# stsievert/pytorch-ps-mpi

Measured on AMD Instinct MI355X. Metric: samples/sec (node) ResNet-50 async PS at 1/2/4/8 MI355X; grad bytes/step, higher is better.
Workload: dtype bf16

## Files before the change

### hipps/csrc/bindings.cpp

```cpp
#include <torch/extension.h>
#include <vector>

namespace hipps {
void aggregate(const std::vector<at::Tensor>& slots, at::Tensor acc, double gscale, bool accumulate, bool acquire);
void copy_acquire(at::Tensor src, at::Tensor dst);
void convert(at::Tensor src, at::Tensor dst, double scale);
void gather_flat(const std::vector<at::Tensor>& srcs, at::Tensor table, at::Tensor dst, double scale);
void transpose_cast(at::Tensor src, at::Tensor dst, at::Tensor tiles);
void sgd_step(const std::vector<at::Tensor>& grads, double gscale, at::Tensor p, c10::optional<at::Tensor> buf,
              c10::optional<at::Tensor> pub, bool zero_src, double lr, double wd, double momentum, double dampening,
              bool nesterov, bool first, c10::optional<at::Tensor> mask, c10::optional<at::Tensor> csteps,
              double lookahead);
void adam_step(const std::vector<at::Tensor>& grads, double gscale, at::Tensor p, at::Tensor exp_avg,
               at::Tensor exp_avg_sq, c10::optional<at::Tensor> max_exp_avg_sq, c10::optional<at::Tensor> pub,
               bool zero_src, double lr, double beta1, double beta2, double eps, double wd, int64_t step,
               bool amsgrad, bool torch_mode, c10::optional<at::Tensor> mask, c10::optional<at::Tensor> csteps);
void q8_encode(at::Tensor x, c10::optional<at::Tensor> resid, at::Tensor q, at::Tensor scales, bool stochastic,
               int64_t seed);
void q8_aggregate(const std::vector<at::Tensor>& qs, const std::vector<at::Tensor>& ss, at::Tensor acc, double gscale,
                  bool accumulate, bool acquire);
void topk_encode(at::Tensor g, c10::optional<at::Tensor> resid, int64_t k, at::Tensor idx, at::Tensor val,
                 at::Tensor workspace);
int64_t topk_workspace_bytes(int64_t n, int64_t k);
void topk_accumulate(at::Tensor idx, at::Tensor val, at::Tensor acc, double gscale, bool acquire);
// ... 23 lines not shown
void bn_backward_partials(at::Tensor part, int64_t nrb, at::Tensor dy, at::Tensor x, int64_t mask_mode,
                          at::Tensor weight, at::Tensor mean, at::Tensor invstd, at::Tensor scale, at::Tensor shift,
                          at::Tensor dx, c10::optional<at::Tensor> dres, at::Tensor dweight, at::Tensor dbias, int64_t C,
                          c10::optional<at::Tensor> mask_in, int64_t unr);
int64_t conv1x1_mtiles(int64_t M);
void conv1x1_forward(at::Tensor x, at::Tensor w, at::Tensor y, c10::optional<at::Tensor> part, int64_t Hi,
                     int64_t Wi, int64_t stride, c10::optional<at::Tensor> add, c10::optional<at::Tensor> add_mask,
                     c10::optional<at::Tensor> bn_x, c10::optional<at::Tensor> bn_bits,
                     c10::optional<at::Tensor> bn_mean, c10::optional<at::Tensor> bn_invstd,
                     c10::optional<at::Tensor> bn_scale, c10::optional<at::Tensor> bn_shift,
                     c10::optional<at::Tensor> pro_scale, c10::optional<at::Tensor> pro_shift);
void bn_dual_forward(at::Tensor part3, int64_t nrb3, at::Tensor partd, int64_t nrbd, at::Tensor x3, at::Tensor xd,
                     at::Tensor z, at::Tensor mask, at::Tensor w3, at::Tensor b3, at::Tensor rm3, at::Tensor rv3,
                     at::Tensor mean3, at::Tensor invstd3, at::Tensor scale3, at::Tensor shift3, at::Tensor wd,
                     at::Tensor bd, at::Tensor rmd, at::Tensor rvd, at::Tensor meand, at::Tensor invstdd,
                     at::Tensor scaled, at::Tensor shiftd, int64_t C, double eps3, double mom3, double epsd,
                     double momd);
void bn_dual_backward(c10::optional<at::Tensor> part3, int64_t nrb3, at::Tensor dz, at::Tensor x3, at::Tensor xd,
                      at::Tensor mask, at::Tensor w3, at::Tensor mean3, at::Tensor invstd3, at::Tensor wd,
                      at::Tensor meand, at::Tensor invstdd, at::Tensor dx3, at::Tensor dxd, at::Tensor dw3,
                      at::Tensor db3, at::Tensor dwd, at::Tensor dbd, int64_t C, int64_t unr);
at::Tensor gemm2_dgrad_s2(at::Tensor dy, at::Tensor wf, at::Tensor dx, int64_t bm, int64_t bn,
                          c10::optional<at::Tensor> bn_x, c10::optional<at::Tensor> bn_bits,
                          c10::optional<at::Tensor> bn_mean, c10::optional<at::Tensor> bn_invstd,
                          c10::optional<at::Tensor> bn_scale, c10::optional<at::Tensor> bn_shift);
int64_t gemm2_mtiles(int64_t M, int64_t N, int64_t K, int64_t bm);
void gemm2_conv(at::Tensor x, at::Tensor w, at::Tensor y, c10::optional<at::Tensor> part,
                c10::optional<at::Tensor> add, c10::optional<at::Tensor> add_mask, int64_t Hi, int64_t Wi,
                int64_t stride, int64_t KH, int64_t KW, int64_t pad, int64_t bm, int64_t bn,
                c10::optional<at::Tensor> bn_x, c10::optional<at::Tensor> bn_bits, c10::optional<at::Tensor> bn_mean,
                c10::optional<at::Tensor> bn_invstd, c10::optional<at::Tensor> bn_scale,
                c10::optional<at::Tensor> bn_shift, int64_t stages, bool add_s2,
                c10::optional<at::Tensor> pro_scale, c10::optional<at::Tensor> pro_shift,
                c10::optional<at::Tensor> bias, c10::optional<at::Tensor> gelu_pre, int64_t gelu);
void gemm2_wgrad(at::Tensor dy, at::Tensor x, at::Tensor dw, int64_t KH, int64_t KW, int64_t stride, int64_t pad,
                 int64_t Hi, int64_t Wi, int64_t cfg, int64_t stages,
                 c10::optional<at::Tensor> pro_scale, c10::optional<at::Tensor> pro_shift, int64_t sdiv);
void maxpool3s2_forward(at::Tensor x, at::Tensor y, at::Tensor code, c10::optional<at::Tensor> scale,
                        c10::optional<at::Tensor> shift);
void bn_finalize_partials(at::Tensor part, int64_t nrb, int64_t M, at::Tensor weight, at::Tensor bias,
                          c10::optional<at::Tensor> running_mean, c10::optional<at::Tensor> running_var,
                          at::Tensor mean, at::Tensor invstd, at::Tensor scale, at::Tensor shift, int64_t C, double eps,
                          double momentum);
void maxpool3s2_backward(at::Tensor dy, at::Tensor code, at::Tensor dx);
std::vector<at::Tensor> xent_forward(at::Tensor logits, at::Tensor labels, int64_t ignore_index);
void colsum_fold(at::Tensor part, at::Tensor out);
void colsum_bf16(at::Tensor x, at::Tensor out);
std::vector<at::Tensor> attn_forward(at::Tensor q, at::Tensor k, at::Tensor v, bool causal, double scale,
                                     c10::optional<at::Tensor> kvlen);
std::vector<at::Tensor> attn_backward(at::Tensor dout, at::Tensor q, at::Tensor k, at::Tensor v, at::Tensor o,
                                      at::Tensor lse, bool causal, double scale, c10::optional<at::Tensor> kvlen,
                                      c10::optional<at::Tensor> dq_out, c10::optional<at::Tensor> dk_out,
                                      c10::optional<at::Tensor> dv_out);
void swiglu_forward(at::Tensor a, at::Tensor b, at::Tensor c);
void ln_forward(at::Tensor x, at::Tensor w, at::Tensor b, at::Tensor y, at::Tensor mean, at::Tensor rstd, double eps);
void ln_backward(at::Tensor dy, at::Tensor x, at::Tensor mean, at::Tensor rstd, at::Tensor w, at::Tensor dx,
                 at::Tensor dw, at::Tensor db, c10::optional<at::Tensor> dxsum);
void embed_forward(at::Tensor ids, c10::optional<at::Tensor> tt, at::Tensor word, at::Tensor pos, at::Tensor typ,
                   at::Tensor out);
void embed_pos_backward(at::Tensor dout, at::Tensor dpos, int64_t B, int64_t S);
void embed_seg_backward(at::Tensor dout, at::Tensor sid, at::Tensor perm, at::Tensor dtab);
void rms_forward(at::Tensor x, at::Tensor w, at::Tensor y, at::Tensor rstd, double eps, c10::optional<at::Tensor> add,
                 c10::optional<at::Tensor> xsum);
void rms_backward(at::Tensor dy, at::Tensor x, at::Tensor rstd, at::Tensor w, at::Tensor dx, at::Tensor dw,
                  c10::optional<at::Tensor> dres, c10::optional<at::Tensor> dx16);
void swiglu_backward(at::Tensor g, at::Tensor a, at::Tensor b, at::Tensor da, at::Tensor db);
void rope_apply(at::Tensor x, at::Tensor y, at::Tensor cs, at::Tensor sn, int64_t S, int64_t hd, double sign);
// ... 74 lines not shown
        py::arg("acc"), py::arg("gscale"), py::arg("acquire") = false);
  m.def("topk_q8_accumulate", &hipps::topk_q8_accumulate, "acc[idx] += gscale * deq(q)", py::arg("idx"), py::arg("q"),
        py::arg("scales"), py::arg("acc"), py::arg("gscale"), py::arg("acquire") = false);
  m.def("topk_q8_residual", &hipps::topk_q8_residual, "EF: r[idx] += v - deq(q)");
  m.def("thresh_encode", &hipps::thresh_encode, "variable-size |x|>tau sparsification, device count header");
  m.def("thresh_accumulate", &hipps::thresh_accumulate, "acc[idx[:count]] += gscale * val[:count]", py::arg("count"),
        py::arg("idx"), py::arg("val"), py::arg("acc"), py::arg("gscale"), py::arg("acquire") = false);
  m.def("copy_counted", &hipps::copy_counted, "copy a [count | idx | val] message moving only count entries");
  m.def("bn_forward_train", &hipps::bn_forward_train, "fused channels-last BN train fwd (+res) (+relu)");
  m.def("bn_apply", &hipps::bn_apply, "y = act(x*scale + shift (+res))");
  m.def("bn_backward", &hipps::bn_backward, "fused BN bwd with relu-mask recompute (+dres)");
  m.def("bn_forward_partials", &hipps::bn_forward_partials, "BN fwd finalize+apply from producer-reduced partials");
  m.def("bn_backward_partials", &hipps::bn_backward_partials, "BN bwd finalize+apply from consumer-reduced partials",
        py::arg("part"), py::arg("nrb"), py::arg("dy"), py::arg("x"), py::arg("mask_mode"), py::arg("weight"),
        py::arg("mean"), py::arg("invstd"), py::arg("scale"), py::arg("shift"), py::arg("dx"), py::arg("dres"),
        py::arg("dweight"), py::arg("dbias"), py::arg("C"), py::arg("mask_in"), py::arg("unr") = 0);
  m.def("conv1x1_mtiles", &hipps::conv1x1_mtiles);
  m.def("bn_dual_forward", &hipps::bn_dual_forward,
        "z = relu(bn3(x3) + bnd(xd)) from producer partials: two finalizes + one apply (downsample block)");
  m.def("bn_dual_backward", &hipps::bn_dual_backward,
        "backward of bn_dual_forward: dx3 + the downsample BN's reduction in one pass, then dxd",
        py::arg("part3"), py::arg("nrb3"), py::arg("dz"), py::arg("x3"), py::arg("xd"), py::arg("mask"), py::arg("w3"),
        py::arg("mean3"), py::arg("invstd3"), py::arg("wd"), py::arg("meand"), py::arg("invstdd"), py::arg("dx3"),
        py::arg("dxd"), py::arg("dw3"), py::arg("db3"), py::arg("dwd"), py::arg("dbd"), py::arg("C"),
        py::arg("unr") = 4);
  m.def("gemm2_mtiles", &hipps::gemm2_mtiles, py::arg("M"), py::arg("N"), py::arg("K"), py::arg("bm") = 0);
  m.def("gemm2_conv", &hipps::gemm2_conv, "second-generation MFMA conv GEMM (LDS-DMA staged, 256-row tiles)",
        py::arg("x"), py::arg("w"), py::arg("y"), py::arg("part") = py::none(), py::arg("add") = py::none(),
        py::arg("add_mask") = py::none(), py::arg("Hi"), py::arg("Wi"), py::arg("stride") = 1, py::arg("KH") = 1,
        py::arg("KW") = 1, py::arg("pad") = 0, py::arg("bm") = 0, py::arg("bn") = 0, py::arg("bn_x") = py::none(),
        py::arg("bn_bits") = py::none(), py::arg("bn_mean") = py::none(), py::arg("bn_invstd") = py::none(),
        py::arg("bn_scale") = py::none(), py::arg("bn_shift") = py::none(), py::arg("stages") = 2,
        py::arg("add_s2") = false, py::arg("pro_scale") = py::none(), py::arg("pro_shift") = py::none(),
        py::arg("bias") = py::none(), py::arg("gelu_pre") = py::none(), py::arg("gelu") = 0);
  m.def("gemm2_dgrad_s2", &hipps::gemm2_dgrad_s2,
        "stride-2 3x3 input gradient as four output-parity implicit GEMMs (+ BN-backward reduction)",
        py::arg("dy"), py::arg("wf"), py::arg("dx"), py::arg("bm") = 128, py::arg("bn") = 128,
        py::arg("bn_x") = py::none(), py::arg("bn_bits") = py::none(), py::arg("bn_mean") = py::none(),
        py::arg("bn_invstd") = py::none(), py::arg("bn_scale") = py::none(), py::arg("bn_shift") = py::none());
  m.def("gemm2_wgrad", &hipps::gemm2_wgrad, "conv weight gradient on the LDS-DMA MFMA core (split-M slabs)",
        py::arg("dy"), py::arg("x"), py::arg("dw"), py::arg("KH"), py::arg("KW"), py::arg("stride"), py::arg("pad"),
        py::arg("Hi"), py::arg("Wi"), py::arg("cfg") = 0, py::arg("stages") = 2, py::arg("pro_scale") = py::none(),
        py::arg("pro_shift") = py::none(), py::arg("sdiv") = 1);
  m.def("conv1x1_forward", &hipps::conv1x1_forward,
        "MFMA 1x1 conv (NHWC GEMM) with fused BN-stats epilogue and optional (+ add * mask) epilogue",
        pybind11::arg("x"), pybind11::arg("w"), pybind11::arg("y"), pybind11::arg("part"), pybind11::arg("Hi"),
        pybind11::arg("Wi"), pybind11::arg("stride"), pybind11::arg("add") = pybind11::none(),
        pybind11::arg("add_mask") = pybind11::none(), pybind11::arg("bn_x") = pybind11::none(),
        pybind11::arg("bn_bits") = pybind11::none(), pybind11::arg("bn_mean") = pybind11::none(),
        pybind11::arg("bn_invstd") = pybind11::none(), pybind11::arg("bn_scale") = pybind11::none(),
        pybind11::arg("bn_shift") = pybind11::none(), pybind11::arg("pro_scale") = pybind11::none(),
        pybind11::arg("pro_shift") = pybind11::none());
  m.def("convkxk_forward", &hipps::convkxk_forward,
        "MFMA KxK conv forward (implicit GEMM, channels-last bf16) with optional BN-statistics epilogue",
        pybind11::arg("x"), pybind11::arg("w"), pybind11::arg("y"), pybind11::arg("part") = pybind11::none(),
        pybind11::arg("stride") = 1, pybind11::arg("pad") = 1);
  m.def("stem_mtiles", &hipps::stem_mtiles, "number of BN partial-statistic columns of stem_forward");
  m.def("stem_forward", &hipps::stem_forward,
        "ResNet stem 7x7/s2/p3 3->64 conv forward on MFMA (channels-last bf16), optional BN-statistics epilogue",
        pybind11::arg("x"), pybind11::arg("w"), pybind11::arg("y"), pybind11::arg("part") = pybind11::none());
  m.def("stem_bnpool_backward", &hipps::stem_bnpool_backward,
        "backward of maxpool(relu(bn(stem(x)))): BN parameter grads + stem weight grad, no pool gradient "
        "materialised (the BN input gradient only with materialize_dy)",
        py::arg("dp"), py::arg("code"), py::arg("y"), py::arg("x"), py::arg("bn_weight"), py::arg("mean"),
        py::arg("invstd"), py::arg("scale"), py::arg("shift"), py::arg("dbn_w"), py::arg("dbn_b"), py::arg("dw"),
        py::arg("materialize_dy") = false, py::arg("quad") = true);
  m.def("stem_wgrad", &hipps::stem_wgrad, "ResNet stem 7x7/s2/p3 weight gradient on MFMA (fp32 dW, deterministic)");
// ... 82 lines not shown
```

### hipps/csrc/gemm2.hip

```cpp
#include "common.h"

#include <ATen/ATen.h>
#include <cstdlib>
#include <mutex>
#include <c10/hip/HIPStream.h>
#include <torch/extension.h>

namespace hipps {
namespace g2 {

typedef short bf16x8 __attribute__((ext_vector_type(8)));
typedef float f32x4 __attribute__((ext_vector_type(4)));
typedef float f32x16 __attribute__((ext_vector_type(16)));
typedef uint32_t u32x4 __attribute__((ext_vector_type(4)));
typedef __attribute__((address_space(3))) void lds_void;
typedef __attribute__((address_space(1))) void glb_void;

constexpr int BK = 64;

__device__ __attribute__((aligned(64))) const uint16_t kZero16[32] = {0};
__device__ __attribute__((aligned(64))) const uint8_t kOnes8[64] = {
    0xff, 0xff, 0xff, 0xff, 0xff, 0xff, 0xff, 0xff, 0xff, 0xff, 0xff, 0xff, 0xff, 0xff, 0xff, 0xff,
    0xff, 0xff, 0xff, 0xff, 0xff, 0xff, 0xff, 0xff, 0xff, 0xff, 0xff, 0xff, 0xff, 0xff, 0xff, 0xff,
    0xff, 0xff, 0xff, 0xff, 0xff, 0xff, 0xff, 0xff, 0xff, 0xff, 0xff, 0xff, 0xff, 0xff, 0xff, 0xff,
    0xff, 0xff, 0xff, 0xff, 0xff, 0xff, 0xff, 0xff, 0xff, 0xff, 0xff, 0xff, 0xff, 0xff, 0xff, 0xff};

enum Epi : int { kPlain = 0, kStats = 1, kAdd = 2, kBst = 4, kBstBits = 8, kAddS2 = 16, kPar = 32, kPro = 64,
                 kBias = 128, kGelu = 256, kGeluB = 512, kGeluBS = 1024 };

__device__ __forceinline__ float erf_fast(float z, float& ez2) {
  const float az = fabsf(z);
  const float t = __builtin_amdgcn_rcpf(fmaf(0.3275911f, az, 1.f));
  ez2 = __expf(-az * az);
  float p = fmaf(1.061405429f, t, -1.453152027f);
  p = fmaf(p, t, 1.421413741f);
  p = fmaf(p, t, -0.284496736f);
  p = fmaf(p, t, 0.254829592f);
  const float e = fmaf(-p * t, ez2, 1.f);
  return copysignf(e, z);
}
__device__ __forceinline__ float gelu_f(float x) {
  float ez2;
  return x * 0.5f * (1.f + erf_fast(x * 0.70710678118654752f, ez2));
}
__device__ __forceinline__ float gelu_bwd_f(float dy, float x) {
  float ez2;
  const float cdf = 0.5f * (1.f + erf_fast(x * 0.70710678118654752f, ez2));
  return dy * fmaf(x, 0.3989422804014327f * ez2, cdf);
}

template <int BM, int BN> struct Cfg;
template <> struct Cfg<256, 256> { static constexpr int TM = 128, TN = 64; };
template <> struct Cfg<256, 128> { static constexpr int TM = 64, TN = 64; };
template <> struct Cfg<128, 128> { static constexpr int TM = 64, TN = 64; };
template <> struct Cfg<256, 64> { static constexpr int TM = 64, TN = 64; };
template <> struct Cfg<128, 64> { static constexpr int TM = 64, TN = 32; };

template <int BM, int BN> constexpr int nthreads() { return 64 * (BM / Cfg<BM, BN>::TM) * (BN / Cfg<BM, BN>::TN); }

template <int BM, int BN, int NS = 2> constexpr int lds_bytes() {
  constexpr int stage = (NS >= 4 ? 2 : NS) * (BM + BN) * BK * 2;
  constexpr int epi = BM * (BN + 8) * 2;
  constexpr int wm = BM / Cfg<BM, BN>::TM;
  return (stage > epi ? stage : epi) + 2 * 2 * wm * BN * 4;
}

struct Args {
  const uint16_t* X;
  const uint16_t* W;
  uint16_t* Y;
  float* pa;
  float* pb;
  const uint16_t* R;
  const uint8_t* RM;
  const uint16_t* bx;
  const uint8_t* bbits;
  const float *bmean, *binvstd, *bscale, *bshift;
  int M, N, K, Ho, Wo, Hi, Wi, stride, mtiles, ntiles;
  int KW, pad, Cin;
  int ldb;
  int pstride, pcol0;
  int ph, pw, Hx, Wx;
  int tdr[4], tdc[4], tko[4];
  const float *psc, *psh;
  const float* bias;
  uint16_t* Y2;
  int epf;
};

__device__ __forceinline__ uint32_t add_bf16x2(uint32_t a, uint32_t b) {
  return pack_bf16x2(__uint_as_float(a << 16) + __uint_as_float(b << 16),
                     __uint_as_float(a & 0xffff0000u) + __uint_as_float(b & 0xffff0000u));
}

__device__ __forceinline__ void glds16(const void* src, void* dst) {
  __builtin_amdgcn_global_load_lds((glb_void*)src, (lds_void*)dst, 16, 0, 0);
}

constexpr int waitcnt_vm(int n) { return (n & 15) | ((n >> 4) << 14) | (7 << 4) | (15 << 8); }
constexpr int waitcnt_lgkm(int n) { return 15 | (3 << 14) | (7 << 4) | ((n & 15) << 8); }

__host__ __device__ constexpr int khalf_swz(int row) {
  return ((0x1320 >> (4 * ((row >> 2) & 3))) & 3);
}

template <int BM, int BN, int EPI, bool TAPS, int NS>
__global__ __launch_bounds__((nthreads<BM, BN>())) void k_gemm(Args g) {
  constexpr int TM = Cfg<BM, BN>::TM, TN = Cfg<BM, BN>::TN;
  constexpr int WM = BM / TM, WN = BN / TN, NW = WM * WN, NT = 64 * NW;
  constexpr int FM = TM / 16, FN = TN / 16;
  constexpr bool KH = NS == 4;
  constexpr bool PP = NS == 5;
  constexpr bool M32 = NS == 6;
  constexpr int NSX = M32 ? 2 : NS;
  constexpr bool PAR = (EPI & kPar) != 0;
  constexpr bool PRO = (EPI & kPro) != 0;
  static_assert(!PAR || TAPS, "kPar needs the implicit-GEMM loader");
  static_assert(!PRO || NS == 2, "kPro: 2 LDS stages");
  static_assert(!PP || (BM == 256 && BN == 256), "ping-pong: 256x256 on 8 waves");
  static_assert(!M32 || (BM == 256 && BN == 256 && !PRO), "32x32x16 MFMA: the 256x256 tile");
  auto orow = [&](int m) -> int64_t {
    if constexpr (PAR) {
      const int hw = g.Ho * g.Wo;
      const int img = m / hw, rem = m - img * hw;
      const int a = rem / g.Wo, b = rem - a * g.Wo;
      return ((int64_t)img * g.Hx + 2 * a + g.ph) * g.Wx + 2 * b + g.pw;
    } else {
      return m;
    }
  };
  constexpr int STAGE = (BM + BN) * BK;
  constexpr int UNIT = (BM + BN) * 32;
  constexpr int RPI = KH ? 16 : 8;
// ... 602 lines not shown
    float* red = reinterpret_cast<float*>(lds);
    __syncthreads();
#pragma unroll
    for (int j = 0; j < 8; ++j) {
      red[(t / RCH) * BN + cc + j] = bsa[j];
      red[RL * BN + (t / RCH) * BN + cc + j] = bsb[j];
    }
    __syncthreads();
    if (t < BN) {
      float sa = 0.f, sb = 0.f;
      for (int r = 0; r < RL; ++r) {
        sa += red[r * BN + t];
        sb += red[RL * BN + r * BN + t];
      }
      if constexpr (GBS) {
        g.pa[(int64_t)mt * g.N + n0 + t] = sa;
      } else {
        g.pa[(int64_t)(n0 + t) * g.pstride + g.pcol0 + mt] = sa;
        g.pb[(int64_t)(n0 + t) * g.pstride + g.pcol0 + mt] = sb;
      }
    }
  }
  if (STATS && t < BN) {
    float sa = 0.f, qa = 0.f;
#pragma unroll
    for (int i = 0; i < WM; ++i) {
      sa += st[(i * BN + t) * 2];
      qa += st[(i * BN + t) * 2 + 1];
    }
    g.pa[(int64_t)(n0 + t) * g.pstride + g.pcol0 + mt] = sa;
    g.pb[(int64_t)(n0 + t) * g.pstride + g.pcol0 + mt] = qa;
  }
}

struct FastDiv2 {
  uint32_t d, mul, shift;
};
inline FastDiv2 make_fastdiv2(uint32_t d) {
  uint32_t l = 0;
  while ((1ull << l) < d) ++l;
  const uint64_t mul = ((((1ull << l) - d) << 32) / d) + 1;
  return FastDiv2{d, (uint32_t)mul, l};
}
__device__ __forceinline__ uint32_t fdiv2(uint32_t n, const FastDiv2& f) { return (__umulhi(n, f.mul) + n) >> f.shift; }

struct WArgs {
  const uint16_t* dY;
  const uint16_t* X;
  float* part;
  int M, N, K, Cin, Ho, Wo, Hi, Wi, stride, KW, pad, chunk, tn, tk;
  FastDiv2 fd_hw, fd_w;
  const float *psc, *psh;
  int* cnt;
  int S, G;
  float* dw;
};

typedef short s16x4 __attribute__((ext_vector_type(4)));

template <int TW>
__device__ __forceinline__ int wswz(int row) {
  return TW >= 128 ? (((row & 3) << 2) | ((row >> 2) & 3)) : (((row & 3) << 1) | ((row >> 2) & 1));
}

template <int TW>
__device__ __forceinline__ bf16x8 tr_frag2(const uint8_t* tile, int row0, int col0, int lane) {
  const int il = lane & 15, q = il >> 2, p = il & 3;
  const int r = row0 + 8 * (lane >> 4) + q;
  const int ch = (col0 >> 3) + (p >> 1);
  typedef __attribute__((address_space(3))) s16x4 lds_s16x4;
  const s16x4 lo = __builtin_amdgcn_ds_read_tr16_b64_v4i16(
      (lds_s16x4*)(tile + 2 * TW * r + 16 * (ch ^ wswz<TW>(r)) + 8 * (p & 1)));
  const s16x4 hi = __builtin_amdgcn_ds_read_tr16_b64_v4i16(
      (lds_s16x4*)(tile + 2 * TW * (r + 4) + 16 * (ch ^ wswz<TW>(r + 4)) + 8 * (p & 1)));
  return __builtin_shufflevector(lo, hi, 0, 1, 2, 3, 4, 5, 6, 7);
}

// ... 302 lines not shown
      } else {
        tot.x += r.x; tot.y += r.y; tot.z += r.z; tot.w += r.w;
      }
    }
    *reinterpret_cast<float4*>(g.dw + (int64_t)n * g.K + k) = tot;
  }
}

inline void pick_tile(int64_t M, int64_t N, int64_t K, int& bm, int& bn) {
  auto blocks = [&](int a, int b) { return ((M + a - 1) / a) * (N / b); };
  if (N % 256 == 0 && ((K >= 1024 && blocks(256, 256) >= 192 && blocks(128, 128) < 1536) ||
                       (K >= 2048 && blocks(256, 256) >= 512))) {
    bm = 256; bn = 256; return;
  }
  if (N % 128 == 0) { bm = 128; bn = 128; return; }
  bm = 128; bn = 64;
}

}

int64_t gemm2_mtiles(int64_t M, int64_t N, int64_t K, int64_t bm) {
  int b = (int)bm, n = 0;
  if (b <= 0) g2::pick_tile(M, N, K, b, n);
  return (M + b - 1) / b;
}

void gemm2_conv(at::Tensor x, at::Tensor w, at::Tensor y, c10::optional<at::Tensor> part,
                c10::optional<at::Tensor> add, c10::optional<at::Tensor> add_mask, int64_t Hi, int64_t Wi,
                int64_t stride, int64_t KH, int64_t KW, int64_t pad, int64_t bm, int64_t bn,
                c10::optional<at::Tensor> bn_x, c10::optional<at::Tensor> bn_bits, c10::optional<at::Tensor> bn_mean,
                c10::optional<at::Tensor> bn_invstd, c10::optional<at::Tensor> bn_scale,
                c10::optional<at::Tensor> bn_shift, int64_t stages, bool add_s2,
                c10::optional<at::Tensor> pro_scale, c10::optional<at::Tensor> pro_shift,
                c10::optional<at::Tensor> bias, c10::optional<at::Tensor> gelu_pre, int64_t gelu) {
  TORCH_CHECK(x.is_cuda() && w.is_cuda() && y.is_cuda(), "gemm2: device tensors");
  TORCH_CHECK(stages >= 2 && stages <= 6,
              "gemm2: stages must be 2, 3, 4 (k-half units), 5 (ping-pong) or 6 (32x32x16 MFMA)");
  TORCH_CHECK(x.scalar_type() == at::kBFloat16 && w.scalar_type() == at::kBFloat16 &&
                  y.scalar_type() == at::kBFloat16, "gemm2: bf16 tensors");
  const int64_t N = w.size(0), K = w.numel() / N, Cin = K / (KH * KW);
  TORCH_CHECK(Cin * KH * KW == K && Cin % g2::BK == 0 && N % 64 == 0, "gemm2: needs Cin % 64 == 0, Cout % 64 == 0");
  const int64_t imgs = x.numel() / (Cin * Hi * Wi);
  TORCH_CHECK(imgs * Cin * Hi * Wi == x.numel(), "gemm2: x size");
  const int64_t Ho = (Hi + 2 * pad - KH) / stride + 1, Wo = (Wi + 2 * pad - KW) / stride + 1;
  const int64_t M = imgs * Ho * Wo;
  TORCH_CHECK(y.numel() == M * N, "gemm2: y size");
  TORCH_CHECK(w.is_contiguous() || w.is_contiguous(at::MemoryFormat::ChannelsLast), "gemm2: dense w");
  for (const at::Tensor* t : {&x, &w, &y})
    TORCH_CHECK(reinterpret_cast<uintptr_t>(t->data_ptr()) % 16 == 0, "gemm2: 16-byte aligned tensors");
  TORCH_CHECK(x.dim() != 4 || x.is_contiguous(at::MemoryFormat::ChannelsLast), "gemm2: channels-last x");
  TORCH_CHECK(y.dim() != 4 || y.is_contiguous(at::MemoryFormat::ChannelsLast), "gemm2: channels-last y");
  TORCH_CHECK(w.dim() != 4 || KH * KW == 1 || w.is_contiguous(at::MemoryFormat::ChannelsLast), "gemm2: channels-last w");
  TORCH_CHECK(M < (int64_t(1) << 31) && x.numel() < (int64_t(1) << 40), "gemm2: size");
  int BMv = (int)bm, BNv = (int)bn;
  if (BMv <= 0 || BNv <= 0) g2::pick_tile(M, N, K, BMv, BNv);
  TORCH_CHECK(N % BNv == 0, "gemm2: Cout must be a multiple of the block tile");
  const int64_t mtiles = (M + BMv - 1) / BMv, ntiles = N / BNv;
  TORCH_CHECK(mtiles * ntiles < (int64_t(1) << 31), "gemm2: grid");
  g2::Args a{};
  a.X = (const uint16_t*)x.data_ptr();
  a.W = (const uint16_t*)w.data_ptr();
  a.Y = (uint16_t*)y.data_ptr();
  a.M = (int)M; a.N = (int)N; a.K = (int)K; a.Ho = (int)Ho; a.Wo = (int)Wo; a.Hi = (int)Hi; a.Wi = (int)Wi;
  a.stride = (int)stride; a.mtiles = (int)mtiles; a.ntiles = (int)ntiles;
  a.KW = (int)KW; a.pad = (int)pad; a.Cin = (int)Cin;
  a.ldb = (int)K; a.pstride = (int)mtiles; a.pcol0 = 0;
  int epi = g2::kPlain;
// ... 61 lines not shown
  }
  if (gelu_pre.has_value() && gelu_pre->defined()) {
    TORCH_CHECK(epi == g2::kPlain && !taps && (gelu == 1 || gelu == 2),
                "gemm2: the GELU epilogues run on a plain 1x1 GEMM (gelu=1 forward, 2 backward)");
    TORCH_CHECK(gelu_pre->is_cuda() && gelu_pre->scalar_type() == at::kBFloat16 && gelu_pre->numel() == M * N &&
                    gelu_pre->is_contiguous() && reinterpret_cast<uintptr_t>(gelu_pre->data_ptr()) % 16 == 0,
                "gemm2: gelu_pre must be a 16-byte aligned contiguous bf16 tensor shaped like y");
    if (gelu == 1) {
      a.Y2 = (uint16_t*)gelu_pre->data_ptr();
      epi |= g2::kGelu;
    } else {
      TORCH_CHECK(!(bias.has_value() && bias->defined()), "gemm2: the GELU backward epilogue takes no bias");
      a.bx = (const uint16_t*)gelu_pre->data_ptr();
      epi |= g2::kGeluB;
      if (a.pa != nullptr) epi |= g2::kGeluBS;
    }
  } else {
    TORCH_CHECK(gelu == 0, "gemm2: gelu needs gelu_pre");
  }
  if (bias.has_value() && bias->defined()) {
    TORCH_CHECK((epi == g2::kPlain || epi == g2::kAdd || epi == g2::kGelu) && !taps,
                "gemm2: the bias epilogue runs on a 1x1 GEMM, alone or with a plain add (a residual)");
    TORCH_CHECK(bias->is_cuda() && bias->scalar_type() == at::kFloat && bias->is_contiguous() && bias->numel() == N,
                "gemm2: bias must be f32 [Cout]");
    a.bias = bias->data_ptr<float>();
    epi |= g2::kBias;
  }
  static const int epf_env = [] {
    const char* e = std::getenv("HIPPS_G2_EPF");
    return e ? std::atoi(e) : 1;
  }();
  a.epf = epf_env;
  auto stream = c10::hip::getCurrentHIPStream();
  const int grid = (int)(mtiles * ntiles);
#define HIPPS_G2S(BMc, BNc, EPc, TPc, NSc) \
  hipLaunchKernelGGL((g2::k_gemm<BMc, BNc, EPc, TPc, NSc>), grid, (g2::nthreads<BMc, BNc>()), 0, stream, a)
#define HIPPS_G2(BMc, BNc, EPc, TPc) \
  do {                                                      \
    if (NS3) HIPPS_G2S(BMc, BNc, EPc, TPc, NS3_OF(BMc, BNc)); \
    else if (NS4) HIPPS_G2S(BMc, BNc, EPc, TPc, 4);          \
    else if (NS5) HIPPS_G2S(BMc, BNc, EPc, TPc, NS5_OF(BMc, BNc)); \
    else if (NS6) HIPPS_G2S(BMc, BNc, EPc, TPc, NS6_OF(BMc, BNc)); \
    else HIPPS_G2S(BMc, BNc, EPc, TPc, 2);                   \
  } while (0)
#define HIPPS_G2_E(BMc, BNc)                                                                        \
  do {                                                                                              \
    if (taps) {                                                                                     \
      switch (epi) {                                                                                \
        case g2::kStats | g2::kPro: HIPPS_G2S(BMc, BNc, (g2::kStats | g2::kPro), true, 2); break;    \
        case g2::kStats: HIPPS_G2(BMc, BNc, g2::kStats, true); break;                               \
        case g2::kBst: HIPPS_G2(BMc, BNc, g2::kBst, true); break;                                   \
        case g2::kBstBits: HIPPS_G2(BMc, BNc, g2::kBstBits, true); break;                           \
        default: HIPPS_G2(BMc, BNc, g2::kPlain, true); break;                                       \
      }                                                                                             \
    } else {                                                                                        \
      switch (epi) {                                                                                \
        case g2::kStats | g2::kPro: HIPPS_G2S(BMc, BNc, (g2::kStats | g2::kPro), false, 2); break;   \
        case g2::kStats: HIPPS_G2(BMc, BNc, g2::kStats, false); break;                              \
        case g2::kAdd: HIPPS_G2(BMc, BNc, g2::kAdd, false); break;                                  \
        case g2::kBias: HIPPS_G2(BMc, BNc, g2::kBias, false); break;                                \
        case g2::kBias | g2::kAdd: HIPPS_G2(BMc, BNc, (g2::kBias | g2::kAdd), false); break;        \
        case g2::kGelu: HIPPS_G2(BMc, BNc, g2::kGelu, false); break;                                \
        case g2::kBias | g2::kGelu: HIPPS_G2(BMc, BNc, (g2::kBias | g2::kGelu), false); break;      \
        case g2::kGeluB: HIPPS_G2(BMc, BNc, g2::kGeluB, false); break;                              \
        case g2::kGeluB | g2::kGeluBS: HIPPS_G2(BMc, BNc, (g2::kGeluB | g2::kGeluBS), false); break;  \
        case g2::kBst: HIPPS_G2(BMc, BNc, g2::kBst, false); break;                                  \
// ... 285 lines not shown
```

Measured before the change: 12200.

## Add persistent halo-ring 3x3 conv kernel for 64-channel stride-1 layers

Adds a specialised persistent kernel for 3x3/stride-1/pad-1 64->64 channel convolutions. Each workgroup keeps all nine weight taps resident in LDS and streams input rows into an LDS ring buffer with a padded halo layout. All nine taps then read from that one staged window instead of re-gathering im2col tiles for each tap. It is enabled by default when the shape fits, with an env var and argument to disable it. The cost is a large LDS footprint (lower occupancy), a grid capped at the CU count, and a new hand-scheduled code path that carries correctness risk.

```diff
diff --git a/hipps/csrc/bindings.cpp b/hipps/csrc/bindings.cpp
--- a/hipps/csrc/bindings.cpp
+++ b/hipps/csrc/bindings.cpp
@@ -79,7 +79,8 @@
                 c10::optional<at::Tensor> bn_invstd, c10::optional<at::Tensor> bn_scale,
                 c10::optional<at::Tensor> bn_shift, int64_t stages, bool add_s2,
                 c10::optional<at::Tensor> pro_scale, c10::optional<at::Tensor> pro_shift,
-                c10::optional<at::Tensor> bias, c10::optional<at::Tensor> gelu_pre, int64_t gelu);
+                c10::optional<at::Tensor> bias, c10::optional<at::Tensor> gelu_pre, int64_t gelu, int64_t halo,
+                int64_t halo_grid);
 void gemm2_wgrad(at::Tensor dy, at::Tensor x, at::Tensor dw, int64_t KH, int64_t KW, int64_t stride, int64_t pad,
                  int64_t Hi, int64_t Wi, int64_t cfg, int64_t stages,
                  c10::optional<at::Tensor> pro_scale, c10::optional<at::Tensor> pro_shift, int64_t sdiv);
@@ -220,7 +221,8 @@
         py::arg("bn_bits") = py::none(), py::arg("bn_mean") = py::none(), py::arg("bn_invstd") = py::none(),
         py::arg("bn_scale") = py::none(), py::arg("bn_shift") = py::none(), py::arg("stages") = 2,
         py::arg("add_s2") = false, py::arg("pro_scale") = py::none(), py::arg("pro_shift") = py::none(),
-        py::arg("bias") = py::none(), py::arg("gelu_pre") = py::none(), py::arg("gelu") = 0);
+        py::arg("bias") = py::none(), py::arg("gelu_pre") = py::none(), py::arg("gelu") = 0, py::arg("halo") = -1,
+        py::arg("halo_grid") = 0);
   m.def("gemm2_dgrad_s2", &hipps::gemm2_dgrad_s2,
         "stride-2 3x3 input gradient as four output-parity implicit GEMMs (+ BN-backward reduction)",
         py::arg("dy"), py::arg("wf"), py::arg("dx"), py::arg("bm") = 128, py::arg("bn") = 128,
diff --git a/hipps/csrc/gemm2.hip b/hipps/csrc/gemm2.hip
--- a/hipps/csrc/gemm2.hip
+++ b/hipps/csrc/gemm2.hip
@@ -1,6 +1,8 @@
 #include "common.h"
+#include "gemm2_common.h"
 
 #include <ATen/ATen.h>
+#include <algorithm>
 #include <cstdlib>
 #include <mutex>
 #include <c10/hip/HIPStream.h>
@@ -9,24 +11,13 @@
 namespace hipps {
 namespace g2 {
 
-typedef short bf16x8 __attribute__((ext_vector_type(8)));
-typedef float f32x4 __attribute__((ext_vector_type(4)));
-typedef float f32x16 __attribute__((ext_vector_type(16)));
-typedef uint32_t u32x4 __attribute__((ext_vector_type(4)));
-typedef __attribute__((address_space(3))) void lds_void;
-typedef __attribute__((address_space(1))) void glb_void;
-
 constexpr int BK = 64;
 
-__device__ __attribute__((aligned(64))) const uint16_t kZero16[32] = {0};
 __device__ __attribute__((aligned(64))) const uint8_t kOnes8[64] = {
     0xff, 0xff, 0xff, 0xff, 0xff, 0xff, 0xff, 0xff, 0xff, 0xff, 0xff, 0xff, 0xff, 0xff, 0xff, 0xff,
     0xff, 0xff, 0xff, 0xff, 0xff, 0xff, 0xff, 0xff, 0xff, 0xff, 0xff, 0xff, 0xff, 0xff, 0xff, 0xff,
     0xff, 0xff, 0xff, 0xff, 0xff, 0xff, 0xff, 0xff, 0xff, 0xff, 0xff, 0xff, 0xff, 0xff, 0xff, 0xff,
     0xff, 0xff, 0xff, 0xff, 0xff, 0xff, 0xff, 0xff, 0xff, 0xff, 0xff, 0xff, 0xff, 0xff, 0xff, 0xff};
-
-enum Epi : int { kPlain = 0, kStats = 1, kAdd = 2, kBst = 4, kBstBits = 8, kAddS2 = 16, kPar = 32, kPro = 64,
-                 kBias = 128, kGelu = 256, kGeluB = 512, kGeluBS = 1024 };
 
 __device__ __forceinline__ float erf_fast(float z, float& ez2) {
   const float az = fabsf(z);
@@ -92,13 +83,6 @@
   return pack_bf16x2(__uint_as_float(a << 16) + __uint_as_float(b << 16),
                      __uint_as_float(a & 0xffff0000u) + __uint_as_float(b & 0xffff0000u));
 }
-
-__device__ __forceinline__ void glds16(const void* src, void* dst) {
-  __builtin_amdgcn_global_load_lds((glb_void*)src, (lds_void*)dst, 16, 0, 0);
-}
-
-constexpr int waitcnt_vm(int n) { return (n & 15) | ((n >> 4) << 14) | (7 << 4) | (15 << 8); }
-constexpr int waitcnt_lgkm(int n) { return 15 | (3 << 14) | (7 << 4) | ((n & 15) << 8); }
 
 __host__ __device__ constexpr int khalf_swz(int row) {
   return ((0x1320 >> (4 * ((row >> 2) & 3))) & 3);
@@ -767,17 +751,6 @@
     g.pb[(int64_t)(n0 + t) * g.pstride + g.pcol0 + mt] = qa;
   }
 }
-
-struct FastDiv2 {
-  uint32_t d, mul, shift;
-};
-inline FastDiv2 make_fastdiv2(uint32_t d) {
-  uint32_t l = 0;
-  while ((1ull << l) < d) ++l;
-  const uint64_t mul = ((((1ull << l) - d) << 32) / d) + 1;
-  return FastDiv2{d, (uint32_t)mul, l};
-}
-__device__ __forceinline__ uint32_t fdiv2(uint32_t n, const FastDiv2& f) { return (__umulhi(n, f.mul) + n) >> f.shift; }
 
 struct WArgs {
   const uint16_t* dY;
@@ -1146,7 +1119,8 @@
                 c10::optional<at::Tensor> bn_invstd, c10::optional<at::Tensor> bn_scale,
                 c10::optional<at::Tensor> bn_shift, int64_t stages, bool add_s2,
                 c10::optional<at::Tensor> pro_scale, c10::optional<at::Tensor> pro_shift,
-                c10::optional<at::Tensor> bias, c10::optional<at::Tensor> gelu_pre, int64_t gelu) {
+                c10::optional<at::Tensor> bias, c10::optional<at::Tensor> gelu_pre, int64_t gelu, int64_t halo,
+                int64_t halo_grid) {
   TORCH_CHECK(x.is_cuda() && w.is_cuda() && y.is_cuda(), "gemm2: device tensors");
   TORCH_CHECK(stages >= 2 && stages <= 6,
               "gemm2: stages must be 2, 3, 4 (k-half units), 5 (ping-pong) or 6 (32x32x16 MFMA)");
@@ -1274,6 +1248,42 @@
   }();
   a.epf = epf_env;
   auto stream = c10::hip::getCurrentHIPStream();
+  {
+    static const int halo_env = [] {
+      const char* e = std::getenv("HIPPS_G2_HALO");
+      return e ? std::atoi(e) : 1;
+    }();
+    TORCH_CHECK(halo >= -1 && halo <= 1 && halo_grid >= 0, "gemm2: halo is -1 (auto), 0 or 1; halo_grid >= 0");
+    const bool shape_ok = KH == 3 && KW == 3 && stride == 1 && pad == 1 && Cin == 64 && N == 64 && BMv == 128 &&
+                          BNv == 64 && stages == 2 &&
+                          (epi == g2::kPlain || epi == g2::kStats || epi == g2::kBst || epi == g2::kBstBits);
+    if (halo == 1) {
+      TORCH_CHECK(shape_ok, "gemm2: halo=1 needs a 3x3 / stride 1 / pad 1 conv of 64 -> 64 channels on the 128x64 "
+                            "tile with 2 stages and a plain, statistics or BN-backward epilogue");
+      TORCH_CHECK(g2::halo3x3_fits(imgs, Hi, Wi), "gemm2: halo=1: the window of a ", Hi, " x ", Wi,
+                  " image does not fit the LDS ring");
+    }
+    if (halo == 1 || (halo == -1 && halo_env != 0 && shape_ok && g2::halo3x3_fits(imgs, Hi, Wi))) {
+      static const int ncu = [] {
+        int dev = 0, n = 0;
+        if (hipGetDevice(&dev) != hipSuccess ||
+            hipDeviceGetAttribute(&n, hipDeviceAttributeMultiprocessorCount, dev) != hipSuccess || n <= 0)
+          n = 256;
+        return n;
+      }();
+      g2::HaloArgs h{};
+      h.X = a.X; h.W = a.W; h.Y = a.Y; h.pa = a.pa; h.pb = a.pb; h.bx = a.bx; h.bbits = a.bbits;
+      h.bmean = a.bmean; h.binvstd = a.binvstd; h.bscale = a.bscale; h.bshift = a.bshift;
+      h.M = (int)M; h.imgs = (int)imgs; h.H = (int)Hi; h.Wd = (int)Wi; h.mtiles = (int)mtiles;
+      h.fd_hw = g2::make_fastdiv2((uint32_t)(Hi * Wi));
+      h.fd_w = g2::make_fastdiv2((uint32_t)Wi);
+      h.fd_p = g2::make_fastdiv2((uint32_t)(Wi + 1));
+      h.fd_h1 = g2::make_fastdiv2((uint32_t)(Hi + 1));
+      const int64_t cap = halo_grid > 0 ? halo_grid : ncu;
+      g2::halo3x3_launch(h, epi, (int)std::min<int64_t>(mtiles, cap), stream);
+      return;
+    }
+  }
   const int grid = (int)(mtiles * ntiles);
 #define HIPPS_G2S(BMc, BNc, EPc, TPc, NSc) \
   hipLaunchKernelGGL((g2::k_gemm<BMc, BNc, EPc, TPc, NSc>), grid, (g2::nthreads<BMc, BNc>()), 0, stream, a)
diff --git a/hipps/csrc/gemm2_common.h b/hipps/csrc/gemm2_common.h
--- /dev/null
+++ b/hipps/csrc/gemm2_common.h
@@ -0,0 +1,54 @@
+#pragma once
+
+#include "common.h"
+
+namespace hipps {
+namespace g2 {
+
+typedef short bf16x8 __attribute__((ext_vector_type(8)));
+typedef float f32x4 __attribute__((ext_vector_type(4)));
+typedef float f32x16 __attribute__((ext_vector_type(16)));
+typedef uint32_t u32x4 __attribute__((ext_vector_type(4)));
+typedef __attribute__((address_space(3))) void lds_void;
+typedef __attribute__((address_space(1))) void glb_void;
+
+__device__ __attribute__((aligned(64))) const uint16_t kZero16[32] = {0};
+
+enum Epi : int { kPlain = 0, kStats = 1, kAdd = 2, kBst = 4, kBstBits = 8, kAddS2 = 16, kPar = 32, kPro = 64,
+                 kBias = 128, kGelu = 256, kGeluB = 512, kGeluBS = 1024 };
+
+__device__ __forceinline__ void glds16(const void* src, void* dst) {
+  __builtin_amdgcn_global_load_lds((glb_void*)src, (lds_void*)dst, 16, 0, 0);
+}
+
+constexpr int waitcnt_vm(int n) { return (n & 15) | ((n >> 4) << 14) | (7 << 4) | (15 << 8); }
+constexpr int waitcnt_lgkm(int n) { return 15 | (3 << 14) | (7 << 4) | ((n & 15) << 8); }
+
+struct FastDiv2 {
+  uint32_t d, mul, shift;
+};
+inline FastDiv2 make_fastdiv2(uint32_t d) {
+  uint32_t l = 0;
+  while ((1ull << l) < d) ++l;
+  const uint64_t mul = ((((1ull << l) - d) << 32) / d) + 1;
+  return FastDiv2{d, (uint32_t)mul, l};
+}
+__device__ __forceinline__ uint32_t fdiv2(uint32_t n, const FastDiv2& f) { return (__umulhi(n, f.mul) + n) >> f.shift; }
+
+struct HaloArgs {
+  const uint16_t* X;
+  const uint16_t* W;
+  uint16_t* Y;
+  float* pa;
+  float* pb;
+  const uint16_t* bx;
+  const uint8_t* bbits;
+  const float *bmean, *binvstd, *bscale, *bshift;
+  int M, imgs, H, Wd, mtiles;
+  FastDiv2 fd_hw, fd_w, fd_p, fd_h1;
+};
+bool halo3x3_fits(int64_t imgs, int64_t H, int64_t W);
+void halo3x3_launch(const HaloArgs& a, int epi, int grid, hipStream_t stream);
+
+}
+}
diff --git a/hipps/csrc/gemm2_halo.hip b/hipps/csrc/gemm2_halo.hip
--- /dev/null
+++ b/hipps/csrc/gemm2_halo.hip
@@ -0,0 +1,344 @@
+#include "gemm2_common.h"
+
+#include <algorithm>
+#include <c10/util/Exception.h>
+#include <map>
+#include <mutex>
+#include <tuple>
+#include <utility>
+
+namespace hipps {
+namespace g2 {
+
+namespace halo {
+constexpr int BM = 128, BN = 64, C = 64, KT = 9 * C;
+constexpr int RING = 512;
+constexpr int TAPB = BN * C * 2;
+constexpr int EP = BN + 8;
+constexpr int L_RING = 8 * TAPB;
+constexpr int L_W8 = L_RING + RING * 128;
+constexpr int L_EPI = L_W8 + TAPB;
+constexpr int L_ST = L_EPI + BM * EP * 2;
+constexpr int L_END = L_ST + 2 * 2 * 2 * BN * 4;
+static_assert(L_END <= 160 * 1024, "LDS budget");
+constexpr int wts_off(int tap) { return tap < 8 ? tap * TAPB : L_W8; }
+}
+
+template <class F, int... I>
+__device__ __forceinline__ void sfor_impl(F&& f, std::integer_sequence<int, I...>) {
+  (f(std::integral_constant<int, I>{}), ...);
+}
+template <int N, class F>
+__device__ __forceinline__ void sfor(F&& f) {
+  sfor_impl(f, std::make_integer_sequence<int, N>{});
+}
+
+template <int EPI>
+__global__ __launch_bounds__(256) void k_halo3x3(HaloArgs g) {
+  using namespace halo;
+  constexpr int TM = 64, TN = 32, WM = 2, NT = 256, FM = TM / 16, FN = TN / 16;
+  constexpr bool STATS = (EPI & kStats) != 0;
+  constexpr int BST = (EPI & kBstBits) ? 2 : (EPI & kBst) ? 1 : 0;
+  __shared__ __attribute__((aligned(16))) uint8_t lds[L_END];
+
+  const int nwg = gridDim.x;
+  const int t0 = (int)((int64_t)blockIdx.x * g.mtiles / nwg), t1 = (int)((int64_t)(blockIdx.x + 1) * g.mtiles / nwg);
+  if (t0 >= t1) return;
+  const int t = threadIdx.x, lane = t & 63;
+  const int w = __builtin_amdgcn_readfirstlane(t >> 6);
+  const int wm = w >> 1, wn = w & 1;
+  const int P = g.Wd + 1, H1 = g.H + 1;
+  auto qpos = [&](int m) -> int {
+    return m + (int)fdiv2((uint32_t)m, g.fd_w) + (int)fdiv2((uint32_t)m, g.fd_hw) * P + P + 1;
+  };
+  const int lr = lane >> 3, lc8 = ((lane & 7) ^ lr) * 8;
+  auto stage = [&](int k0, int k1) {
+    for (int k = k0 + w; k < k1; k += 4) {
+      const int p = 8 * k + lr;
+      const int r = (int)fdiv2((uint32_t)p, g.fd_p), c = p - r * P;
+      const int ri = (int)fdiv2((uint32_t)r, g.fd_h1), rh = r - ri * H1;
+      const bool ok = c != 0 && rh != 0 && ri < g.imgs;
+      const int m = p - r - (ri + 1) * g.Wd - 1;
+      const uint16_t* src = ok ? g.X + (int64_t)m * C + lc8 : kZero16;
+      glds16(src, lds + L_RING + ((8 * k) & (RING - 1)) * 128);
+    }
+  };
+
+  for (int e = w; e < 72; e += 4) {
+    const int tap = e >> 3, rg = e & 7;
+    glds16(g.W + (rg * 8 + lr) * KT + tap * C + lc8, lds + (tap < 8 ? tap * TAPB : L_W8) + rg * 1024);
+  }
+  int hi;
+  {
+    const int m0 = t0 * BM, ml = m0 + BM - 1 < g.M ? m0 + BM - 1 : g.M - 1;
+    hi = qpos(ml) + P + 1;
+    stage((qpos(m0) - P - 1) >> 3, (hi >> 3) + 1);
+  }
+  int b_off[2][FN], b_off8[2][FN];
+#pragma unroll
+  for (int j = 0; j < FN; ++j) {
+    const int n = wn * TN + j * 16 + (lane & 15);
+    b_off[0][j] = n * 128 + (((lane >> 4) ^ (n & 7)) << 4);
+    b_off[1][j] = b_off[0][j] ^ 64;
+    b_off8[0][j] = b_off[0][j] + L_W8;
+    b_off8[1][j] = b_off[1][j] + L_W8;
+  }
+  const int c4 = ((lane >> 4) << 4) | L_RING;
+  constexpr int RCH = BN / 8, NOUT = BM * RCH / NT;
+  const int cc = (t % RCH) * 8;
+  float bmu[8], bis[8], bsc[8], bsh[8];
+  if (BST) {
+#pragma unroll
+    for (int j = 0; j < 8; ++j) {
+      bmu[j] = g.bmean[cc + j];
+      bis[j] = g.binvstd[cc + j];
+      bsc[j] = BST == 1 ? g.bscale[cc + j] : 0.f;
+      bsh[j] = BST == 1 ? g.bshift[cc + j] : 0.f;
+    }
+  }
+
+  __builtin_amdgcn_s_waitcnt(waitcnt_vm(0));
+  for (int mt = t0; mt < t1; ++mt) {
+    const int m0 = mt * BM;
+    int qa4[FM];
+    {
+      const int m = m0 + wm * TM + lane;
+      const int q4 = qpos(m < g.M ? m : g.M - 1) << 4;
+#pragma unroll
+      for (int i = 0; i < FM; ++i) qa4[i] = __shfl(q4, i * 16 + (lane & 15), 64);
+    }
+    asm volatile("" ::: "memory");
+    __builtin_amdgcn_s_waitcnt(waitcnt_lgkm(0));
+    __builtin_amdgcn_s_barrier();
+    asm volatile("" ::: "memory");
+    if (mt + 1 < t1) {
+      const int ml = m0 + 2 * BM - 1 < g.M ? m0 + 2 * BM - 1 : g.M - 1;
+      const int nhi = qpos(ml) + P + 1;
+      stage((hi >> 3) + 1, (nhi >> 3) + 1);
+      hi = nhi;
+    }
+    u32x4 px[BST ? NOUT : 1];
+    uint32_t pxm[BST ? NOUT : 1];
+    if constexpr (BST != 0) {
+#pragma unroll
+      for (int i = 0; i < NOUT; ++i) {
+        const int id = t + NT * i;
+        const int row = id / RCH, c = id - row * RCH;
+        const int64_t o = (int64_t)(m0 + row < g.M ? m0 + row : m0) * BN + c * 8;
+        px[i] = *reinterpret_cast<const u32x4*>(g.bx + o);
+        pxm[i] = BST == 2 ? g.bbits[o >> 3] : 0u;
+      }
+    }
+
+    f32x4 acc[FM][FN];
+#pragma unroll
+    for (int i = 0; i < FM; ++i)
+#pragma unroll
+      for (int j = 0; j < FN; ++j) acc[i][j] = f32x4{0.f, 0.f, 0.f, 0.f};
+    bf16x8 fa[2][2][FM], fb[2][2][FN];
+    int ad[2][FM], ah[2][FM];
+    auto addr_step = [&](auto tapc, auto gc) {
+      constexpr int tap = decltype(tapc)::value, g4 = decltype(gc)::value, set = tap & 1, i = g4 >> 2;
+      if constexpr ((g4 & 3) == 0) {
+        ad[set][i] = qa4[i] + ((tap / 3 - 1) * P + (tap % 3 - 1)) * 16;
+        ah[set][i] = ad[set][i] << 3;
+      } else if constexpr ((g4 & 3) == 1) {
+        ah[set][i] &= (RING - 1) * 128;
+      } else if constexpr ((g4 & 3) == 2) {
+        ad[set][i] = ah[set][i] | ((ad[set][i] & 0x70) ^ c4);
+      } else {
+        ah[set][i] = ad[set][i] ^ 64;
+      }
+    };
+    auto gap_work = [&fa, &fb, &ad, &ah, &b_off, &b_off8, &addr_step](auto tapc, auto gc) {
+      constexpr int tap = decltype(tapc)::value, g4 = decltype(gc)::value, set = tap & 1;
+      if constexpr (tap + 1 < 9) addr_step(std::integral_constant<int, tap + 1>{}, gc);
+      if constexpr ((g4 & 3) != 3) {
+        constexpr int u = g4 - g4 / 4, ks = u / 6, v = u % 6;
+        if constexpr (v < 2) {
+          asm volatile("ds_read_b128 %0, %1 offset:%2"
+                       : "=v"(fb[set][ks][v])
+                       : "v"(tap < 8 ? b_off[ks][v] : b_off8[ks][v]), "n"(tap < 8 ? tap * TAPB : 0));
+        } else {
+          asm volatile("ds_read_b128 %0, %1" : "=v"(fa[set][ks][v - 2]) : "v"(ks ? ah[set][v - 2] : ad[set][v - 2]));
+        }
+      }
+    };
+    sfor<16>([&](auto gc) { addr_step(std::integral_constant<int, 0>{}, gc); });
+    sfor<16>([&](auto gc) { gap_work(std::integral_constant<int, 0>{}, gc); });
+    sfor<9>([&](auto tapc) {
+      constexpr int tap = decltype(tapc)::value;
+      sfor<16>([&](auto uc) {
+        constexpr int u = decltype(uc)::value;
+        constexpr int ks = u >> 3, i = (u >> 1) & 3, j = u & 1;
+        if constexpr (j == 0) {
+          constexpr int need = 6 * ks + 2 + i;
+          constexpr int younger = 11 - need + (tap + 1 < 9 ? u - u / 4 : 0);
+          __builtin_amdgcn_s_waitcnt(waitcnt_lgkm(younger));
+          __builtin_amdgcn_sched_barrier(0);
+        }
+        acc[i][j] = __builtin_amdgcn_mfma_f32_16x16x32_bf16(fa[tap & 1][ks][i], fb[tap & 1][ks][j], acc[i][j], 0, 0, 0);
+        __builtin_amdgcn_sched_barrier(0);
+        if constexpr (tap + 1 < 9) {
+          gap_work(std::integral_constant<int, tap + 1>{}, uc);
+          __builtin_amdgcn_sched_barrier(0);
+        }
+      });
+    });
+    if (m0 + BM > g.M) {
+      asm volatile("" ::: "memory");
+#pragma unroll
+      for (int i = 0; i < FM; ++i)
+#pragma unroll
+        for (int r = 0; r < 4; ++r)
+          if (m0 + wm * TM + i * 16 + (lane >> 4) * 4 + r >= g.M) {
+#pragma unroll
+            for (int j = 0; j < FN; ++j) acc[i][j][r] = 0.f;
+          }
+    }
+
+    uint16_t* ep = reinterpret_cast<uint16_t*>(lds + L_EPI);
+    float* st = reinterpret_cast<float*>(lds + L_ST);
+#pragma unroll
+    for (int j = 0; j < FN; ++j) {
+      const int col = wn * TN + j * 16 + (lane & 15);
+      float s = 0.f, qq = 0.f;
+#pragma unroll
+      for (int i = 0; i < FM; ++i) {
+#pragma unroll
+        for (int r = 0; r < 4; ++r) {
+          const int row = wm * TM + i * 16 + (lane >> 4) * 4 + r;
+          const uint16_t hb = f32_to_bf16(acc[i][j][r]);
+          ep[row * EP + col] = hb;
+          if (STATS) {
+            const float v = bf16_to_f32(hb);
+            s += v;
+            qq = fmaf(v, v, qq);
+          }
+        }
+      }
+      if (STATS) {
+        s += __shfl_xor(s, 16, 64);
+        qq += __shfl_xor(qq, 16, 64);
+        s += __shfl_xor(s, 32, 64);
+        qq += __shfl_xor(qq, 32, 64);
+        if (lane < 16) {
+          st[(wm * BN + col) * 2] = s;
+          st[(wm * BN + col) * 2 + 1] = qq;
+        }
+      }
+    }
+    __builtin_amdgcn_s_waitcnt(waitcnt_vm(0));
+    asm volatile("s_waitcnt lgkmcnt(0)" ::: "memory");
+    __builtin_amdgcn_s_barrier();
+    asm volatile("" ::: "memory");
+    float bsa[8], bsb[8];
+    if (BST) {
+#pragma unroll
+      for (int j = 0; j < 8; ++j) bsa[j] = bsb[j] = 0.f;
+    }
+    uint4 ov[NOUT];
+#pragma unroll
+    for (int i = 0; i < NOUT; ++i) {
+      const int id = t + NT * i;
+      ov[i] = *reinterpret_cast<const uint4*>(ep + (id / RCH) * EP + (id % RCH) * 8);
+    }
+#pragma unroll
+    for (int i = 0; i < NOUT; ++i) {
+      const int id = t + NT * i;
+      const int row = id / RCH, c = id - row * RCH;
+      if (m0 + row < g.M) {
+        const int64_t o = (int64_t)(m0 + row) * BN + c * 8;
+        const uint4 v = ov[i];
+        *reinterpret_cast<uint4*>(g.Y + o) = v;
+        if (BST) {
+          const u32x4 xu = px[BST ? i : 0];
+          const uint32_t mbits = pxm[BST ? i : 0];
+          const uint32_t dv[4] = {v.x, v.y, v.z, v.w};
+          const uint32_t xw[4] = {xu.x, xu.y, xu.z, xu.w};
+#pragma unroll
+          for (int j = 0; j < 8; ++j) {
+            const float d = __uint_as_float(j & 1 ? dv[j >> 1] & 0xffff0000u : dv[j >> 1] << 16);
+            const float xv = __uint_as_float(j & 1 ? xw[j >> 1] & 0xffff0000u : xw[j >> 1] << 16);
+            const bool on = BST == 2 ? ((mbits >> j) & 1u) != 0u : fmaf(xv, bsc[j], bsh[j]) > 0.f;
+            const float dz = on ? d : 0.f;
+            bsa[j] += dz;
+            bsb[j] = fmaf(dz, (xv - bmu[j]) * bis[j], bsb[j]);
+          }
+        }
+      }
+    }
+    if (BST) {
+      constexpr int RL = NT / RCH;
+      static_assert(2 * RL * BN * 4 <= BM * EP * 2, "BST scratch");
+      float* red = reinterpret_cast<float*>(lds + L_EPI);
+      asm volatile("s_waitcnt lgkmcnt(0)" ::: "memory");
+      __builtin_amdgcn_s_barrier();
+      asm volatile("" ::: "memory");
+#pragma unroll
+      for (int j = 0; j < 8; ++j) {
+        red[(t / RCH) * BN + cc + j] = bsa[j];
+        red[RL * BN + (t / RCH) * BN + cc + j] = bsb[j];
+      }
+      asm volatile("s_waitcnt lgkmcnt(0)" ::: "memory");
+      __builtin_amdgcn_s_barrier();
+      asm volatile("" ::: "memory");
+      if (t < 2 * BN) {
+        const int which = t >> 6, ch = t & 63;
+        const float* rp = red + which * RL * BN + ch;
+        float sa = 0.f;
+#pragma unroll
+        for (int r = 0; r < RL; ++r) sa += rp[r * BN];
+        (which ? g.pb : g.pa)[(int64_t)ch * g.mtiles + mt] = sa;
+      }
+    }
+    if (STATS && t < BN) {
+      float sa = 0.f, qa = 0.f;
+#pragma unroll
+      for (int i = 0; i < WM; ++i) {
+        sa += st[(i * BN + t) * 2];
+        qa += st[(i * BN + t) * 2 + 1];
+      }
+      g.pa[(int64_t)t * g.mtiles + mt] = sa;
+      g.pb[(int64_t)t * g.mtiles + mt] = qa;
+    }
+  }
+}
+
+bool halo3x3_fits(int64_t imgs, int64_t H, int64_t W) {
+  static std::mutex mu;
+  static std::map<std::tuple<int64_t, int64_t, int64_t>, bool> seen;
+  const auto key = std::make_tuple(imgs, H, W);
+  std::lock_guard<std::mutex> lk(mu);
+  auto it = seen.find(key);
+  if (it != seen.end()) return it->second;
+  const int64_t P = W + 1, H1 = H + 1, M = imgs * H * W;
+  bool ok = imgs > 0 && H > 0 && W > 0 && M < (int64_t(1) << 31) && (imgs * H1 + 4) * P < (int64_t(1) << 27);
+  if (ok) {
+    auto q = [&](int64_t m) {
+      const int64_t img = m / (H * W), rem = m - img * H * W, h = rem / W, x = rem - h * W;
+      return (img * H1 + h + 1) * P + x + 1;
+    };
+    const int64_t mtiles = (M + halo::BM - 1) / halo::BM;
+    for (int64_t i = 0; i < mtiles && ok; ++i) {
+      const int64_t lo = q(i * halo::BM) - P - 1;
+      const int64_t hi = q(std::min<int64_t>(i * halo::BM + 2 * halo::BM - 1, M - 1)) + P + 1;
+      ok = (hi | 7) - (lo & ~int64_t(7)) + 1 <= halo::RING;
+    }
+  }
+  seen[key] = ok;
+  return ok;
+}
+
+void halo3x3_launch(const HaloArgs& a, int epi, int grid, hipStream_t stream) {
+  switch (epi) {
+    case kPlain: hipLaunchKernelGGL((k_halo3x3<kPlain>), grid, 256, 0, stream, a); break;
+    case kStats: hipLaunchKernelGGL((k_halo3x3<kStats>), grid, 256, 0, stream, a); break;
+    case kBst: hipLaunchKernelGGL((k_halo3x3<kBst>), grid, 256, 0, stream, a); break;
+    case kBstBits: hipLaunchKernelGGL((k_halo3x3<kBstBits>), grid, 256, 0, stream, a); break;
+    default: TORCH_CHECK(false, "gemm2: the halo 3x3 kernel has no epilogue ", epi);
+  }
+}
+
+}
+}
```

Result: slower. 10720 (-12.1%).
